# rrwick/Filtlong

Hardware: AMD Instinct MI355X
Metric: Mbases/s scored+sorted (higher is better)
Workload: dtype f64; 1 GPU; 10,000,000 synthetic reads per GPU x gamma(k=4) mean 10 kbp, Phred-only, --target_bases 50008889515 (50% of bases); C2; reads_total=10000000, bases_total=100017779031, window_size=250, parallelism=1 GPU, device=AMD Radeon Graphics (gfx950:sramecc+:xnack-), gpus_visible=1, cut=select

## Files before the change

filtlong_amd/csrc/score_phred_regs.hip:

```cpp
#include <algorithm>

#include "flx_internal.h"
#include "score_phred_common.h"

using namespace flx_phred;

#ifndef FLX_REGS_PART
#define FLX_REGS_PART 0
#endif

namespace {

template <bool PRIV>
struct Tab {
    static constexpr int ROW = PRIV ? 256 : 8;
    static constexpr int ENTRIES = PRIV ? 129 : LUT_PAD;
    static constexpr int BYTES = ROW * ENTRIES;
    static constexpr int QOFF = 0;
    static constexpr int DOFF = BYTES;
    static constexpr int ZIDX = PRIV ? 128 : 256;
    static constexpr int SLOT0 = 2 * BYTES;
};

template <bool PRIV, int SEL>
__device__ __forceinline__ uint32_t tab_addr(uint32_t x, uint32_t laneoff) {
    if (PRIV) {
        constexpr uint32_t sel = 0x0c0c0000u | ((4u + SEL) << 8);
        return __builtin_amdgcn_perm(x, laneoff, sel);
    }
    return lut_addr(x, SEL);
}
template <bool PRIV>
__device__ __forceinline__ uint32_t tab_addr_at(const uint32_t (&x)[8], int e, uint32_t laneoff) {
    switch (e & 3) {
        case 0: return tab_addr<PRIV, 0>(x[e >> 2], laneoff);
        case 1: return tab_addr<PRIV, 1>(x[e >> 2], laneoff);
        case 2: return tab_addr<PRIV, 2>(x[e >> 2], laneoff);
        default: return tab_addr<PRIV, 3>(x[e >> 2], laneoff);
    }
}

template <int QOFF, int DOFF>
__device__ __forceinline__ void fold4(uint32_t aj0, uint32_t aj1, uint32_t aj2, uint32_t aj3, uint32_t ai0, uint32_t ai1,
                                      uint32_t ai2, uint32_t ai3, double &s, double &w, double &mn) {
    double q0, i0, j0, q1, i1, j1, q2, i2, j2, q3, i3, j3;
    asm volatile(
        "ds_read_b64 %3, %15 offset:%23\n\tds_read_b64 %4, %19 offset:%24\n\tds_read_b64 %5, %15 offset:%24\n\t"
        "ds_read_b64 %6, %16 offset:%23\n\tds_read_b64 %7, %20 offset:%24\n\tds_read_b64 %8, %16 offset:%24\n\t"
        "ds_read_b64 %9, %17 offset:%23\n\tds_read_b64 %10, %21 offset:%24\n\tds_read_b64 %11, %17 offset:%24\n\t"
        "ds_read_b64 %12, %18 offset:%23\n\tds_read_b64 %13, %22 offset:%24\n\tds_read_b64 %14, %18 offset:%24\n\t"
        "s_waitcnt lgkmcnt(11)\n\tv_add_f64 %0, %0, %3\n\t"
        "s_waitcnt lgkmcnt(10)\n\tv_add_f64 %1, %1, -%4\n\t"
        "s_waitcnt lgkmcnt(9)\n\tv_add_f64 %1, %1, %5\n\tv_min_f64 %2, %2, %1\n\t"
        "s_waitcnt lgkmcnt(8)\n\tv_add_f64 %0, %0, %6\n\t"
        "s_waitcnt lgkmcnt(7)\n\tv_add_f64 %1, %1, -%7\n\t"
        "s_waitcnt lgkmcnt(6)\n\tv_add_f64 %1, %1, %8\n\tv_min_f64 %2, %2, %1\n\t"
        "s_waitcnt lgkmcnt(5)\n\tv_add_f64 %0, %0, %9\n\t"
        "s_waitcnt lgkmcnt(4)\n\tv_add_f64 %1, %1, -%10\n\t"
        "s_waitcnt lgkmcnt(3)\n\tv_add_f64 %1, %1, %11\n\tv_min_f64 %2, %2, %1\n\t"
        "s_waitcnt lgkmcnt(2)\n\tv_add_f64 %0, %0, %12\n\t"
        "s_waitcnt lgkmcnt(1)\n\tv_add_f64 %1, %1, -%13\n\t"
        "s_waitcnt lgkmcnt(0)\n\tv_add_f64 %1, %1, %14\n\tv_min_f64 %2, %2, %1"
        : "+v"(s), "+v"(w), "+v"(mn), "=&v"(q0), "=&v"(i0), "=&v"(j0), "=&v"(q1), "=&v"(i1), "=&v"(j1), "=&v"(q2), "=&v"(i2),
          "=&v"(j2), "=&v"(q3), "=&v"(i3), "=&v"(j3)
        : "v"(aj0), "v"(aj1), "v"(aj2), "v"(aj3), "v"(ai0), "v"(ai1), "v"(ai2), "v"(ai3), "i"(QOFF), "i"(DOFF));
}
template <int QOFF>
__device__ __forceinline__ void head4(uint32_t aj0, uint32_t aj1, uint32_t aj2, uint32_t aj3, double &s) {
    double q0, q1, q2, q3;
    asm volatile(
        "ds_read_b64 %1, %5 offset:%9\n\tds_read_b64 %2, %6 offset:%9\n\tds_read_b64 %3, %7 offset:%9\n\t"
        "ds_read_b64 %4, %8 offset:%9\n\t"
        "s_waitcnt lgkmcnt(3)\n\tv_add_f64 %0, %0, %1\n\ts_waitcnt lgkmcnt(2)\n\tv_add_f64 %0, %0, %2\n\t"
        "s_waitcnt lgkmcnt(1)\n\tv_add_f64 %0, %0, %3\n\ts_waitcnt lgkmcnt(0)\n\tv_add_f64 %0, %0, %4"
        : "+v"(s), "=&v"(q0), "=&v"(q1), "=&v"(q2), "=&v"(q3)
        : "v"(aj0), "v"(aj1), "v"(aj2), "v"(aj3), "i"(QOFF));
}
template <int QOFF>
__device__ __forceinline__ void head1(uint32_t aj, double &s) {
    double q;
    asm volatile("ds_read_b64 %1, %2 offset:%3\n\ts_waitcnt lgkmcnt(0)\n\tv_add_f64 %0, %0, %1" : "+v"(s), "=&v"(q) : "v"(aj), "i"(QOFF));
}
template <int QOFF, int DOFF>
__device__ __forceinline__ void fold1(uint32_t aj, uint32_t ai, double &s, double &w, double &mn) {
    double q, i, j;
    asm volatile(
        "ds_read_b64 %3, %6 offset:%8\n\tds_read_b64 %4, %7 offset:%9\n\tds_read_b64 %5, %6 offset:%9\n\t"
        "s_waitcnt lgkmcnt(2)\n\tv_add_f64 %0, %0, %3\n\ts_waitcnt lgkmcnt(1)\n\tv_add_f64 %1, %1, -%4\n\t"
        "s_waitcnt lgkmcnt(0)\n\tv_add_f64 %1, %1, %5\n\tv_min_f64 %2, %2, %1"
        : "+v"(s), "+v"(w), "+v"(mn), "=&v"(q), "=&v"(i), "=&v"(j)
        : "v"(aj), "v"(ai), "i"(QOFF), "i"(DOFF));
}

__device__ __forceinline__ void dma16(const void *gsrc, uint32_t lds_dst) {
    unsigned keep;
    asm volatile("s_mov_b32 %0, m0\n\ts_mov_b32 m0, %2\n\ts_nop 0\n\tglobal_load_lds_dwordx4 %1, off\n\ts_mov_b32 m0, %0"
                 : "=&s"(keep)
                 : "v"(gsrc), "s"(lds_dst)
                 : "memory");
}

__device__ __forceinline__ void funnel(const uint32_t (&p0)[4], const uint32_t (&p1)[4], int fD, uint32_t fsh, uint32_t (&tw)[4]) {
    const uint32_t x[8] = {p0[0], p0[1], p0[2], p0[3], p1[0], p1[1], p1[2], p1[3]};
#define FLX_FUN(D) _Pragma("unroll") for (int d = 0; d < 4; ++d) tw[d] = __builtin_amdgcn_alignbyte(x[(D) + d + 1], x[(D) + d], fsh);
    switch (fD) {
        case 0: FLX_FUN(0) break;
        case 1: FLX_FUN(1) break;
        case 2: FLX_FUN(2) break;
        case 3: FLX_FUN(3) break;
        default: tw[0] = x[4]; tw[1] = x[5]; tw[2] = x[6]; tw[3] = x[7]; break;
    }
#undef FLX_FUN
}

template <int A, bool PRIV, int WAVES, int BS = -1>
__global__ void __launch_bounds__(WAVES * 64) flx_score_phred_regs(const PhredArgs a) {
    using T = Tab<PRIV>;
    if (a.use_private && (*a.use_private != 0u) != PRIV) return;
    constexpr int R = ((A + 5 + 3) / 4) * 4;
    constexpr int RR = R / 4;
    constexpr int H = (A + 1 + 3) / 4;
    constexpr int SLOT_BYTES = 8192;
    static_assert(H <= RR, "prologue must fit one ring revolution");
    extern __shared__ __attribute__((aligned(16))) unsigned char smem[];

    if (PRIV) {
        for (int i = threadIdx.x; i < 129 * 32; i += WAVES * 64) {
            const int e = i >> 5;
            const double q = e < 128 ? a.lut_q[e] : 0.0, d = e < 128 ? a.lut_d[e] : 0.0;
            *reinterpret_cast<double *>(smem + T::QOFF + i * 8) = q;
            *reinterpret_cast<double *>(smem + T::DOFF + i * 8) = d;
        }
    } else {
        for (int i = threadIdx.x; i < 257; i += WAVES * 64) {
            *reinterpret_cast<double *>(smem + T::QOFF + i * 8) = a.lut_q[i];
            *reinterpret_cast<double *>(smem + T::DOFF + i * 8) = a.lut_d[i];
        }
    }
    __syncthreads();

    const int lane = threadIdx.x & 63;
    const int wave = threadIdx.x >> 6;
    unsigned char *slot = smem + T::SLOT0 + wave * SLOT_BYTES;
    const uint32_t slot_lds = (uint32_t)__builtin_amdgcn_readfirstlane((int)(T::SLOT0 + wave * SLOT_BYTES));
    const unsigned char *my_row = slot + lane * 64;
    const int rot = lane >> 2;
    const uint32_t laneoff = (uint32_t)(lane & 31) * 8u;
    const uint32_t zaddr = PRIV ? (uint32_t)(T::ZIDX * T::ROW) + laneoff : (uint32_t)(T::ZIDX * T::ROW);
    const int ws = a.ws;
    const int B = BS >= 0 ? BS : ws & 15;
    const int fD = (16 - B) >> 2;
    const uint32_t fsh = (uint32_t)(16 - B) & 3u;
    const double ws_d = a.ws_d;

  for (;;) {
    unsigned int group = 0;
    if (lane == 0) group = atomicAdd(a.ticket, 1u);
    group = (unsigned int)__builtin_amdgcn_readfirstlane((int)group);
    if (group >= a.n_groups) break;
    const uint64_t gslot = (uint64_t)group * 64 + lane;
    const bool slot_used = gslot < a.n_reads;
    uint32_t rid = 0;
    int L = 0;
    uint64_t base = 0;
    if (slot_used) {
        rid = a.order ? a.order[gslot] : (uint32_t)gslot;
        L = a.lengths[rid];
        base = a.offsets[rid];
    }
    const bool live = slot_used && L < a.long_thr;
    if (!live) L = 0;
    const int Lmax = wave_max(L);
    const int Lmin = wave_min(L);
    if (Lmax == 0) {
        if (live) finish_read(a, rid, L, 0.0, 0.0);
        continue;
    }
    const int n_rounds = (Lmax + 63) >> 6;

    const int dq = ((lane & 3) - (lane >> 4)) & 3;
    const uint8_t *gsrc[4];
    int lim[4];
#pragma unroll
    for (int m = 0; m < 4; ++m) {
        const int r = m * 16 + (lane >> 2);
        const uint32_t lo = __shfl((uint32_t)base, r, 64);
        const uint32_t hi = __shfl((uint32_t)(base >> 32), r, 64);
        gsrc[m] = a.plane + ((((uint64_t)hi << 32) | lo) + (uint64_t)(dq * 16));
        lim[m] = ((__shfl(L, r, 64) + 15) & ~15) - dq * 16;
    }
    auto issue_dma = [&](int c) {
        asm volatile("s_waitcnt lgkmcnt(0)" ::: "memory");
#pragma unroll
        for (int m = 0; m < 4; ++m) {
            const int o = c * 128;
            if (o < lim[m]) dma16(gsrc[m] + o, slot_lds + m * 1024);
            if (o + 64 < lim[m]) dma16(gsrc[m] + o + 64, slot_lds + 4096 + m * 1024);
        }
    };

    uint32_t ring[R][4];
#pragma unroll
    for (int i = 0; i < R; ++i) ring[i][0] = ring[i][1] = ring[i][2] = ring[i][3] = 0;
    double s = 0.0, w = 0.0, mn = 0.0;
    uint32_t bad = 0;

    auto load_round = [&](int t0, int r) {
        const int half = r & 1;
        if (half == 0) asm volatile("s_waitcnt vmcnt(0)" ::: "memory");
        const unsigned char *row = my_row + half * 4096;
#pragma unroll
        for (int k = 0; k < 4; ++k) {
            const uint4 v = *reinterpret_cast<const uint4 *>(row + (((k + rot) & 3) << 4));
            ring[t0 + k][0] = v.x; ring[t0 + k][1] = v.y; ring[t0 + k][2] = v.z; ring[t0 + k][3] = v.w;
            if (PRIV) bad |= v.x | v.y | v.z | v.w;
        }
        if (half == 1 && r + 1 < n_rounds) issue_dma((r + 1) >> 1);
    };
    auto mask4 = [&](bool masked, int rem, int k0, uint32_t (&o)[4]) {
        if (__builtin_expect(masked, 0)) {
#pragma unroll
            for (int i = 0; i < 4; ++i) o[i] = (k0 + i) < rem ? o[i] : zaddr;
        }
    };
    auto addr4 = [&](uint32_t x, bool masked, int rem, int k0, uint32_t (&o)[4]) {
        o[0] = tab_addr<PRIV, 0>(x, laneoff);
        o[1] = tab_addr<PRIV, 1>(x, laneoff);
        o[2] = tab_addr<PRIV, 2>(x, laneoff);
        o[3] = tab_addr<PRIV, 3>(x, laneoff);
        mask4(masked, rem, k0, o);
    };
    auto trail4_static = [&](const uint32_t (&p0)[4], const uint32_t (&p1)[4], int d, bool masked, int rem, uint32_t (&o)[4]) {
        const uint32_t x[8] = {p0[0], p0[1], p0[2], p0[3], p1[0], p1[1], p1[2], p1[3]};
#pragma unroll
        for (int i = 0; i < 4; ++i) o[i] = tab_addr_at<PRIV>(x, 16 - BS + 4 * d + i, laneoff);
        mask4(masked, rem, 4 * d, o);
    };
    auto head_piece = [&](const uint32_t (&lw)[4], int Tp) {
        const bool masked = 16 * (Tp + 1) > Lmin;
        const int rem = L - 16 * Tp;
#pragma unroll
        for (int d = 0; d < 4; ++d) {
            uint32_t aj[4];
            addr4(lw[d], masked, rem, 4 * d, aj);
            head4<T::QOFF>(aj[0], aj[1], aj[2], aj[3], s);
        }
    };
    auto steady_piece = [&](const uint32_t (&lw)[4], const uint32_t (&p0)[4], const uint32_t (&p1)[4], int Tp) {
        const bool masked = 16 * (Tp + 1) > Lmin;
        const int rem = L - 16 * Tp;
        uint32_t tw[4];
        if constexpr (BS < 0) funnel(p0, p1, fD, fsh, tw);
#pragma unroll
        for (int d = 0; d < 4; ++d) {
            uint32_t aj[4], ai[4];
            addr4(lw[d], masked, rem, 4 * d, aj);
            if constexpr (BS < 0) addr4(tw[d], masked, rem, 4 * d, ai);
            else trail4_static(p0, p1, d, masked, rem, ai);
            fold4<T::QOFF, T::DOFF>(aj[0], aj[1], aj[2], aj[3], ai[0], ai[1], ai[2], ai[3], s, w, mn);
        }
    };
    auto boundary_piece = [&](const uint32_t (&lw)[4], const uint32_t (&p0)[4], const uint32_t (&p1)[4], int Tp) {
        const int rem = L - 16 * Tp;
        uint32_t tw[4];
        if constexpr (BS < 0) funnel(p0, p1, fD, fsh, tw);
#pragma unroll
        for (int d = 0; d < 4; ++d) {
            uint32_t aj[4], ai[4];
            addr4(lw[d], true, rem, 4 * d, aj);
            if constexpr (BS < 0) addr4(tw[d], true, rem, 4 * d, ai);
            else trail4_static(p0, p1, d, true, rem, ai);
#pragma unroll
            for (int i = 0; i < 4; ++i) {
                const int k = 4 * d + i;
                if (k < B) head1<T::QOFF>(aj[i], s);
                else fold1<T::QOFF, T::DOFF>(aj[i], ai[i], s, w, mn);
                if (k == B - 1) {
                    w = s / ws_d;
                    mn = w;
                }
            }
        }
    };

    issue_dma(0);

#pragma unroll
    for (int h = 0; h < H; ++h) {
        if (h >= n_rounds) goto done;
        load_round(4 * h, h);
#pragma unroll
        for (int k = 0; k < 4; ++k) {
            constexpr int dummy = 0;
            (void)dummy;
            const int Tp = 4 * h + k;
            if (16 * Tp >= Lmax) continue;
            if (Tp < A) {
                head_piece(ring[Tp], Tp);
                if (Tp == A - 1 && B == 0) {
                    w = s / ws_d;
                    mn = w;
                }
            } else if (Tp == A) {
                boundary_piece(ring[Tp], ring[(Tp + R - A - 1) % R], ring[(Tp + R - A) % R], Tp);
            } else {
                steady_piece(ring[Tp], ring[(Tp + R - A - 1) % R], ring[(Tp + R - A) % R], Tp);
            }
        }
    }
    for (int rb = H;; rb += RR) {
#pragma unroll
        for (int u = 0; u < RR; ++u) {
            const int r = rb + u;
            if (r >= n_rounds) goto done;
            const int sr = (H + u) % RR;
            load_round(4 * sr, r);
#pragma unroll
            for (int k = 0; k < 4; ++k) {
                const int t = 4 * sr + k;
                const int Tp = 4 * r + k;
                if (16 * Tp >= Lmax) break;
                steady_piece(ring[t], ring[(t + R - A - 1) % R], ring[(t + R - A) % R], Tp);
            }
        }
    }
done:
    if (live) {
        finish_read(a, rid, L, s, mn);
        if (PRIV && (bad & 0x80808080u)) a.redo_list[atomicAdd(a.redo_count, 1u)] = rid;
    }
  }
}

#if FLX_REGS_PART == 0
__global__ void __launch_bounds__(1024) flx_score_phred_stream(const PhredArgs a) {
    using T = Tab<false>;
    extern __shared__ __attribute__((aligned(16))) unsigned char smem[];
    for (int i = threadIdx.x; i < 257; i += 1024) {
        *reinterpret_cast<double *>(smem + T::QOFF + i * 8) = a.lut_q[i];
        *reinterpret_cast<double *>(smem + T::DOFF + i * 8) = a.lut_d[i];
    }
    __syncthreads();
    const int lane = threadIdx.x & 63;
    const uint32_t zaddr = (uint32_t)(T::ZIDX * T::ROW);
    const int ws = a.ws;
    const int A = ws >> 4, B = ws & 15;
    const int fD = (16 - B) >> 2;
    const uint32_t fsh = (uint32_t)(16 - B) & 3u;
    const double ws_d = a.ws_d;
    for (;;) {
        unsigned int group = 0;
        if (lane == 0) group = atomicAdd(a.ticket, 1u);
        group = (unsigned int)__builtin_amdgcn_readfirstlane((int)group);
        if (group >= a.n_groups) break;
        const uint64_t gslot = (uint64_t)group * 64 + lane;
        const bool slot_used = gslot < a.n_reads;
        uint32_t rid = 0;
        int L = 0;
        uint64_t base = 0;
        if (slot_used) {
            rid = a.order ? a.order[gslot] : (uint32_t)gslot;
            L = a.lengths[rid];
            base = a.offsets[rid];
        }
        const bool live = slot_used && L < a.long_thr;
        if (!live) L = 0;
        const int Lmax = wave_max(L);
        if (Lmax == 0) {
            if (live) finish_read(a, rid, L, 0.0, 0.0);
            continue;
        }
        const uint8_t *src = (L > 0) ? a.plane + base : a.plane;
        const int maxoff = max(((L + 15) & ~15) - 16, 0);
        auto ld16 = [&](int off) { return *reinterpret_cast<const uint4 *>(src + min(max(off, 0), maxoff)); };
        const int n_pieces = (Lmax + 15) >> 4;
        double s = 0.0, w = 0.0, mn = 0.0;
        uint4 lead = ld16(0), lead_next = ld16(16);
        uint4 tr_prev = make_uint4(0, 0, 0, 0), tr_cur = tr_prev, tr_next = ld16(-16 * A);
        for (int t = 0; t < n_pieces; ++t) {
            const uint4 lw4 = lead;
            lead = lead_next;
            lead_next = ld16(16 * (t + 2));
            tr_prev = tr_cur;
            tr_cur = tr_next;
            tr_next = ld16(16 * (t + 1 - A));
            const uint32_t lw[4] = {lw4.x, lw4.y, lw4.z, lw4.w};
            const int rem = L - 16 * t;
            if (t < A) {
#pragma unroll
                for (int d = 0; d < 4; ++d) {
                    uint32_t aj[4];
                    aj[0] = tab_addr<false, 0>(lw[d], 0); aj[1] = tab_addr<false, 1>(lw[d], 0);
                    aj[2] = tab_addr<false, 2>(lw[d], 0); aj[3] = tab_addr<false, 3>(lw[d], 0);
#pragma unroll
                    for (int i = 0; i < 4; ++i) aj[i] = (4 * d + i) < rem ? aj[i] : zaddr;
                    head4<T::QOFF>(aj[0], aj[1], aj[2], aj[3], s);
                }
                if (t == A - 1 && B == 0) {
                    w = s / ws_d;
                    mn = w;
                }
                continue;
            }
            const uint32_t p0[4] = {tr_prev.x, tr_prev.y, tr_prev.z, tr_prev.w};
            const uint32_t p1[4] = {tr_cur.x, tr_cur.y, tr_cur.z, tr_cur.w};
            uint32_t tw[4];
            funnel(p0, p1, fD, fsh, tw);
#pragma unroll
            for (int d = 0; d < 4; ++d) {
                uint32_t aj[4], ai[4];
                aj[0] = tab_addr<false, 0>(lw[d], 0); aj[1] = tab_addr<false, 1>(lw[d], 0);
                aj[2] = tab_addr<false, 2>(lw[d], 0); aj[3] = tab_addr<false, 3>(lw[d], 0);
                ai[0] = tab_addr<false, 0>(tw[d], 0); ai[1] = tab_addr<false, 1>(tw[d], 0);
                ai[2] = tab_addr<false, 2>(tw[d], 0); ai[3] = tab_addr<false, 3>(tw[d], 0);
#pragma unroll
                for (int i = 0; i < 4; ++i) {
                    const bool act = (4 * d + i) < rem;
                    aj[i] = act ? aj[i] : zaddr;
                    ai[i] = act ? ai[i] : zaddr;
                }
                if (t > A) {
                    fold4<T::QOFF, T::DOFF>(aj[0], aj[1], aj[2], aj[3], ai[0], ai[1], ai[2], ai[3], s, w, mn);
                } else {
#pragma unroll
                    for (int i = 0; i < 4; ++i) {
                        const int k = 4 * d + i;
                        if (k < B) head1<T::QOFF>(aj[i], s);
                        else fold1<T::QOFF, T::DOFF>(aj[i], ai[i], s, w, mn);
                        if (k == B - 1) {
                            w = s / ws_d;
                            mn = w;
                        }
                    }
                }
            }
        }
        if (live) finish_read(a, rid, L, s, mn);
    }
}

constexpr int DUAL_WAVES = 9;
template <int AMOD>
__global__ void __launch_bounds__(DUAL_WAVES * 64) flx_score_phred_dual(const PhredArgs a) {
    using T = Tab<false>;
    constexpr int LEAD_BYTES = 8192, TRAIL_BYTES = 8192, WAVE_BYTES = LEAD_BYTES + TRAIL_BYTES;
    extern __shared__ __attribute__((aligned(16))) unsigned char smem[];
    for (int i = threadIdx.x; i < 257; i += DUAL_WAVES * 64) {
        *reinterpret_cast<double *>(smem + T::QOFF + i * 8) = a.lut_q[i];
        *reinterpret_cast<double *>(smem + T::DOFF + i * 8) = a.lut_d[i];
    }
    __syncthreads();
    const int lane = threadIdx.x & 63;
    const int wave = threadIdx.x >> 6;
    unsigned char *lead_slot = smem + T::SLOT0 + wave * WAVE_BYTES;
    unsigned char *trail_ring = lead_slot + LEAD_BYTES;
    const uint32_t lead_lds = (uint32_t)__builtin_amdgcn_readfirstlane((int)(T::SLOT0 + wave * WAVE_BYTES));
    const uint32_t trail_lds = lead_lds + LEAD_BYTES;
    const int rot = lane >> 2;
    const uint32_t zaddr = (uint32_t)(T::ZIDX * T::ROW);
    const int ws = a.ws;
    const int A = ws >> 4, B = ws & 15;
    const int A4 = A >> 2;
    const int fD = (16 - B) >> 2;
    const uint32_t fsh = (uint32_t)(16 - B) & 3u;
    const double ws_d = a.ws_d;

    for (;;) {
        unsigned int group = 0;
        if (lane == 0) group = atomicAdd(a.ticket, 1u);
        group = (unsigned int)__builtin_amdgcn_readfirstlane((int)group);
        if (group >= a.n_groups) break;
        const uint64_t gslot = (uint64_t)group * 64 + lane;
        const bool slot_used = gslot < a.n_reads;
        uint32_t rid = 0;
        int L = 0;
        uint64_t base = 0;
        if (slot_used) {
            rid = a.order ? a.order[gslot] : (uint32_t)gslot;
            L = a.lengths[rid];
            base = a.offsets[rid];
        }
        const bool live = slot_used && L < a.long_thr;
        if (!live) L = 0;
        const int Lmax = wave_max(L);
        const int Lmin = wave_min(L);
        if (Lmax == 0) {
            if (live) finish_read(a, rid, L, 0.0, 0.0);
            continue;
        }
        const int n_rounds = (Lmax + 63) >> 6;
        const int dq = ((lane & 3) - (lane >> 4)) & 3;
        const uint8_t *gsrc[4];
        int lim[4];
#pragma unroll
        for (int m = 0; m < 4; ++m) {
            const int r = m * 16 + (lane >> 2);
            const uint32_t lo = __shfl((uint32_t)base, r, 64);
            const uint32_t hi = __shfl((uint32_t)(base >> 32), r, 64);
            const int Lr = __shfl(L, r, 64);
            gsrc[m] = Lr > 0 ? a.plane + ((((uint64_t)hi << 32) | lo) + (uint64_t)(dq * 16)) : a.plane;
            lim[m] = Lr > 0 ? ((Lr + 15) & ~15) - dq * 16 : 0;
        }
        auto lds_idle = [&]() { asm volatile("s_waitcnt lgkmcnt(0)" ::: "memory"); };
        auto issue_lead = [&](int c) {
            lds_idle();
            const int o = c * 128;
#pragma unroll
            for (int m = 0; m < 4; ++m) {
                dma16(gsrc[m] + (o < lim[m] ? o : 0), lead_lds + m * 1024);
                dma16(gsrc[m] + (o + 64 < lim[m] ? o + 64 : 0), lead_lds + 4096 + m * 1024);
            }
        };
        auto issue_trail = [&](int h) {
            lds_idle();
            const int o = h * 64;
            const uint32_t dst = trail_lds + (uint32_t)(h & 1) * 4096u;
#pragma unroll
            for (int m = 0; m < 4; ++m) dma16(gsrc[m] + ((o >= 0 && o < lim[m]) ? o : 0), dst + m * 1024);
        };

        double s = 0.0, w = 0.0, mn = 0.0;
        uint32_t prev[4][4];
#pragma unroll
        for (int k = 0; k < 4; ++k) prev[k][0] = prev[k][1] = prev[k][2] = prev[k][3] = 0;
        issue_lead(0);
        if (A4 == 0) issue_trail(0);
        for (int r = 0; r < n_rounds; ++r) {
            const int h = r - A4;
            issue_trail(h + 1);
            asm volatile("s_waitcnt vmcnt(4)" ::: "memory");
            uint32_t lw[4][4], cur[4][4];
            const unsigned char *lrow = lead_slot + (r & 1) * 4096 + lane * 64;
            const unsigned char *trow = trail_ring + (h & 1) * 4096 + lane * 64;
#pragma unroll
            for (int k = 0; k < 4; ++k) {
                const uint4 v = *reinterpret_cast<const uint4 *>(lrow + (((k + rot) & 3) << 4));
                lw[k][0] = v.x; lw[k][1] = v.y; lw[k][2] = v.z; lw[k][3] = v.w;
            }
#pragma unroll
            for (int k = 0; k < 4; ++k) {
                uint4 v = make_uint4(0, 0, 0, 0);
                if (h >= 0) v = *reinterpret_cast<const uint4 *>(trow + (((k + rot) & 3) << 4));
                cur[k][0] = v.x; cur[k][1] = v.y; cur[k][2] = v.z; cur[k][3] = v.w;
            }
            if ((r & 1) && r + 1 < n_rounds) issue_lead((r + 1) >> 1);
#pragma unroll
            for (int k = 0; k < 4; ++k) {
                const int Tp = 4 * r + k;
                if (16 * Tp >= Lmax) break;
                const bool masked = 16 * (Tp + 1) > Lmin;
                const int rem = L - 16 * Tp;
                if (Tp < A) {
#pragma unroll
                    for (int d = 0; d < 4; ++d) {
                        uint32_t aj[4];
                        aj[0] = tab_addr<false, 0>(lw[k][d], 0); aj[1] = tab_addr<false, 1>(lw[k][d], 0);
                        aj[2] = tab_addr<false, 2>(lw[k][d], 0); aj[3] = tab_addr<false, 3>(lw[k][d], 0);
                        if (masked) {
#pragma unroll
                            for (int i = 0; i < 4; ++i) aj[i] = (4 * d + i) < rem ? aj[i] : zaddr;
                        }
                        head4<T::QOFF>(aj[0], aj[1], aj[2], aj[3], s);
                    }
                    if (Tp == A - 1 && B == 0) {
                        w = s / ws_d;
                        mn = w;
                    }
                    continue;
                }
                uint32_t tw[4];
                {
                    constexpr int dummy = 0;
                    (void)dummy;
                    const uint32_t(&p0)[4] = (k <= AMOD) ? prev[3 - AMOD + k] : cur[k - AMOD - 1];
                    const uint32_t(&p1)[4] = (k + 1 <= AMOD) ? prev[3 - AMOD + k + 1] : cur[k - AMOD];
                    funnel(p0, p1, fD, fsh, tw);
                }
#pragma unroll
                for (int d = 0; d < 4; ++d) {
                    uint32_t aj[4], ai[4];
                    aj[0] = tab_addr<false, 0>(lw[k][d], 0); aj[1] = tab_addr<false, 1>(lw[k][d], 0);
                    aj[2] = tab_addr<false, 2>(lw[k][d], 0); aj[3] = tab_addr<false, 3>(lw[k][d], 0);
                    ai[0] = tab_addr<false, 0>(tw[d], 0); ai[1] = tab_addr<false, 1>(tw[d], 0);
                    ai[2] = tab_addr<false, 2>(tw[d], 0); ai[3] = tab_addr<false, 3>(tw[d], 0);
                    if (masked || Tp == A) {
#pragma unroll
                        for (int i = 0; i < 4; ++i) {
                            const bool act = (4 * d + i) < rem;
                            aj[i] = act ? aj[i] : zaddr;
                            ai[i] = act ? ai[i] : zaddr;
                        }
                    }
                    if (Tp > A) {
                        fold4<T::QOFF, T::DOFF>(aj[0], aj[1], aj[2], aj[3], ai[0], ai[1], ai[2], ai[3], s, w, mn);
                    } else {
#pragma unroll
                        for (int i = 0; i < 4; ++i) {
                            const int kk = 4 * d + i;
                            if (kk < B) head1<T::QOFF>(aj[i], s);
                            else fold1<T::QOFF, T::DOFF>(aj[i], ai[i], s, w, mn);
                            if (kk == B - 1) {
                                w = s / ws_d;
                                mn = w;
                            }
                        }
                    }
                }
            }
#pragma unroll
            for (int k = 0; k < 4; ++k) {
                prev[k][0] = cur[k][0]; prev[k][1] = cur[k][1]; prev[k][2] = cur[k][2]; prev[k][3] = cur[k][3];
            }
        }
        asm volatile("s_waitcnt vmcnt(0)" ::: "memory");
        if (live) finish_read(a, rid, L, s, mn);
    }
}

__global__ void __launch_bounds__(256) flx_score_phred_redo(const PhredArgs a) {
    __shared__ double lq[LUT_PAD];
    __shared__ double ld[LUT_PAD];
    for (int i = threadIdx.x; i < 257; i += 256) {
        lq[i] = a.lut_q[i];
        ld[i] = a.lut_d[i];
    }
    __syncthreads();
    const unsigned int n = *a.redo_count;
    for (unsigned int i = blockIdx.x * 256 + threadIdx.x; i < n; i += gridDim.x * 256) {
        const uint32_t rid = a.redo_list[i];
        const int L = a.lengths[rid];
        const uint8_t *q = a.plane + a.offsets[rid];
        const int ws = a.ws;
        double s = 0.0, w = 0.0, mn = 0.0;
        const int head = L < ws ? L : ws;
        for (int j = 0; j < head; ++j) s += lq[q[j]];
        if (L > ws) {
            w = s / a.ws_d;
            mn = w;
            for (int j = ws; j < L; ++j) {
                const uint32_t cj = q[j], ci = q[j - ws];
                s += lq[cj];
                w -= ld[ci];
                w += ld[cj];
                if (w < mn) mn = w;
            }
        }
        finish_read(a, rid, L, s, mn);
    }
}

#endif

template <int A, bool PRIV, int WAVES, int BS = -1>
int launch_one(flx_ctx *ctx, PhredArgs &a) {
    using T = Tab<PRIV>;
    auto kern = flx_score_phred_regs<A, PRIV, WAVES, BS>;
    const size_t lds = std::max<size_t>((size_t)T::SLOT0 + (size_t)WAVES * 8192, 84 * 1024);
    FLX_HIP(ctx, hipFuncSetAttribute((const void *)kern, hipFuncAttributeMaxDynamicSharedMemorySize, (int)lds));
    const uint64_t per_block = (uint64_t)WAVES;
    const unsigned grid = (unsigned)std::min<uint64_t>(((uint64_t)a.n_groups + per_block - 1) / per_block,
                                                       (uint64_t)ctx->prop.multiProcessorCount);
    if (!a.use_private) {
        ctx->last_phred_kernel = PRIV ? "flx_score_phred_regs_private" : "flx_score_phred_regs";
        flx_time_begin(ctx, ctx->last_phred_kernel);
    }
    hipLaunchKernelGGL(kern, dim3(grid), dim3(WAVES * 64), lds, ctx->stream, a);
    if (!a.use_private) flx_time_end(ctx);
    FLX_HIP(ctx, hipGetLastError());
    return FLX_OK;
}

template <int A, bool PRIV>
struct WavesFor {
    static constexpr int plain = A <= 7 ? 16 : A <= 15 ? 12 : 8;
    static constexpr int value = PRIV && plain > 11 ? 11 : plain;
};

template <int A>
int launch_a(flx_ctx *ctx, PhredArgs &a, bool priv, int bs) {
    if constexpr (A == 15) {
        if (bs == 10) return priv ? launch_one<A, true, WavesFor<A, true>::value, 10>(ctx, a) : launch_one<A, false, WavesFor<A, false>::value, 10>(ctx, a);
    }
    if constexpr (A >= 32) {
        return launch_one<A, false, WavesFor<A, false>::value>(ctx, a);
    } else {
        return priv ? launch_one<A, true, WavesFor<A, true>::value>(ctx, a) : launch_one<A, false, WavesFor<A, false>::value>(ctx, a);
    }
}

template <int A, int A_END>
int launch_range(flx_ctx *ctx, PhredArgs &a, bool priv, int bs, bool *launched) {
    if constexpr (A < A_END) {
        if (a.ws / 16 != A) return launch_range<A + 1, A_END>(ctx, a, priv, bs, launched);
        *launched = true;
        return launch_a<A>(ctx, a, priv, bs);
    }
    return FLX_OK;
}

}

#define FLX_REGS_PARTS(X) X(0) X(1) X(2) X(3) X(4) X(5) X(6) X(7)
constexpr int kPartFirstA[] = {0, 8, 13, 18, 23, 28, 32, 36, 39};

#define FLX_REGS_PART_DECL(P) int flx_launch_score_phred_regs_part##P(flx_ctx *ctx, PhredArgs &a, bool priv, int bs, bool *launched);
FLX_REGS_PARTS(FLX_REGS_PART_DECL)
#define FLX_REGS_CAT2(a, b) a##b
#define FLX_REGS_CAT(a, b) FLX_REGS_CAT2(a, b)
int FLX_REGS_CAT(flx_launch_score_phred_regs_part, FLX_REGS_PART)(flx_ctx *ctx, PhredArgs &a, bool priv, int bs, bool *launched) {
    return launch_range<kPartFirstA[FLX_REGS_PART], kPartFirstA[FLX_REGS_PART + 1]>(ctx, a, priv, bs, launched);
}

#if FLX_REGS_PART == 0
namespace {
__global__ void __launch_bounds__(256) flx_phred_sample(const PhredArgs a, unsigned int *hist, unsigned int *done, unsigned int *use_private) {
    const uint64_t t = (uint64_t)blockIdx.x * 256 + threadIdx.x;
    uint64_t z = (t + 1) * 0x9E3779B97F4A7C15ULL;
    z = (z ^ (z >> 30)) * 0xBF58476D1CE4E5B9ULL;
    z = (z ^ (z >> 27)) * 0x94D049BB133111EBULL;
    z ^= z >> 31;
    const uint64_t r = z % a.n_reads;
    const int L = a.lengths[r];
    if (L > 0) {
        const uint32_t pos = (uint32_t)((z >> 32) % (uint64_t)L);
        atomicAdd(&hist[a.plane[a.offsets[r] + pos]], 1u);
    }
    __threadfence();
    __syncthreads();
    if (threadIdx.x != 0 || atomicAdd(done, 1u) != gridDim.x - 1) return;
    __threadfence();
    double tot = 0.0, conflicts = 0.0;
    bool high = false;
    for (int i = 0; i < 256; ++i) {
        const unsigned int h = __hip_atomic_load(&hist[i], __ATOMIC_RELAXED, __HIP_MEMORY_SCOPE_AGENT);
        tot += h;
        high = high || (i >= 128 && h != 0);
    }
    if (tot > 0) {
        for (int b = 0; b < 32; ++b) {
            double pb = 0.0, sq = 0.0;
            for (int e = b; e < 256; e += 32) {
                const double pe = __hip_atomic_load(&hist[e], __ATOMIC_RELAXED, __HIP_MEMORY_SCOPE_AGENT) / tot;
                pb += pe;
                sq += pe * pe;
            }
            conflicts += pb * pb - sq;
        }
    }
    *use_private = (!high && 496.0 * conflicts > 3.0) ? 1u : 0u;
}

}

int flx_launch_score_phred_stream(flx_ctx *ctx, PhredArgs a) {
    void *scr;
    FLX_CHECK(flx_scratch(ctx, 64, &scr));
    FLX_HIP(ctx, hipMemsetAsync(scr, 0, 8, ctx->stream));
    a.ticket = (unsigned int *)scr;
    a.n_groups = (unsigned int)((a.n_reads + 63) / 64);
    const size_t lds = 84 * 1024;
    FLX_HIP(ctx, hipFuncSetAttribute((const void *)flx_score_phred_stream, hipFuncAttributeMaxDynamicSharedMemorySize, (int)lds));
    const unsigned grid = (unsigned)std::min<uint64_t>(((uint64_t)a.n_groups + 15) / 16, (uint64_t)ctx->prop.multiProcessorCount);
    ctx->last_phred_kernel = "flx_score_phred_stream";
    flx_time_begin(ctx, ctx->last_phred_kernel);
    hipLaunchKernelGGL(flx_score_phred_stream, dim3(grid), dim3(1024), lds, ctx->stream, a);
    flx_time_end(ctx);
    FLX_HIP(ctx, hipGetLastError());
    return FLX_OK;
}

int flx_launch_score_phred_dual(flx_ctx *ctx, PhredArgs a) {
    void *scr;
    FLX_CHECK(flx_scratch(ctx, 64, &scr));
    FLX_HIP(ctx, hipMemsetAsync(scr, 0, 8, ctx->stream));
    a.ticket = (unsigned int *)scr;
    a.n_groups = (unsigned int)((a.n_reads + 63) / 64);
    const size_t lds = (size_t)Tab<false>::SLOT0 + (size_t)DUAL_WAVES * 16384;
    const unsigned grid = (unsigned)std::min<uint64_t>(((uint64_t)a.n_groups + DUAL_WAVES - 1) / DUAL_WAVES, (uint64_t)ctx->prop.multiProcessorCount);
    ctx->last_phred_kernel = "flx_score_phred_dual";
    flx_time_begin(ctx, ctx->last_phred_kernel);
#define FLX_DUAL_LAUNCH(M)                                                                                                              \
    case M:                                                                                                                             \
        FLX_HIP(ctx, hipFuncSetAttribute((const void *)flx_score_phred_dual<M>, hipFuncAttributeMaxDynamicSharedMemorySize, (int)lds)); \
        hipLaunchKernelGGL(flx_score_phred_dual<M>, dim3(grid), dim3(DUAL_WAVES * 64), lds, ctx->stream, a);                            \
        break;
    switch ((a.ws >> 4) & 3) {
        FLX_DUAL_LAUNCH(0) FLX_DUAL_LAUNCH(1) FLX_DUAL_LAUNCH(2) FLX_DUAL_LAUNCH(3)
    }
#undef FLX_DUAL_LAUNCH
    flx_time_end(ctx);
    FLX_HIP(ctx, hipGetLastError());
    return FLX_OK;
}

int flx_launch_score_phred_regs(flx_ctx *ctx, PhredArgs a, bool *launched, PhredPending *pd) {
    *launched = false;
    const int A = a.ws / 16;
    constexpr int n_parts = (int)(sizeof kPartFirstA / sizeof kPartFirstA[0]) - 1;
    if (A >= kPartFirstA[n_parts]) return FLX_OK;
    const char *env = getenv("FLX_PHRED_TABLES");
    bool priv = env && strcmp(env, "private") == 0;
    bool forced = env && (strcmp(env, "private") == 0 || strcmp(env, "plain") == 0);
    if (A >= 32) {
        forced = true;
        priv = false;
    }
    const char *fenv = getenv("FLX_PHRED_FUNNEL");
    if (fenv && *fenv && strcmp(fenv, "runtime") != 0)
        return flx_fail(ctx, FLX_ERR_INVALID, "FLX_PHRED_FUNNEL=%s: expected runtime (or unset)", fenv);
    const int bs = (a.ws == 250 && !(fenv && *fenv)) ? 10 : -1;
    void *scr;
    FLX_CHECK(flx_scratch(ctx, 2048 + a.n_reads * 4, &scr));
    a.ticket = (unsigned int *)scr;
    a.redo_count = (unsigned int *)scr + 1;
    a.redo_list = (uint32_t *)((char *)scr + 2048);
    unsigned int *d_flag = (unsigned int *)scr + 3;
    FLX_HIP(ctx, hipMemsetAsync(scr, 0, 2048, ctx->stream));
    if (!forced) {
        hipLaunchKernelGGL(flx_phred_sample, dim3(64), dim3(256), 0, ctx->stream, a, (unsigned int *)((char *)scr + 64),
                           (unsigned int *)scr + 2, d_flag);
        a.use_private = d_flag;
    }
    a.n_groups = (unsigned int)((a.n_reads + 63) / 64);
    typedef int (*part_fn)(flx_ctx *, PhredArgs &, bool, int, bool *);
#define FLX_REGS_PART_NAME(P) flx_launch_score_phred_regs_part##P,
    static const part_fn parts[n_parts] = {FLX_REGS_PARTS(FLX_REGS_PART_NAME)};
#undef FLX_REGS_PART_NAME
    int P = 0;
    while (A >= kPartFirstA[P + 1]) ++P;
    auto part = [&](bool pv) { return parts[P](ctx, a, pv, bs, launched); };
    long timed_index = -1;
    if (forced) {
        FLX_CHECK(part(priv));
    } else {
        ctx->last_phred_kernel = "flx_score_phred_regs";
        flx_time_scope t(ctx, ctx->last_phred_kernel);
        if (ctx->timing) timed_index = (long)ctx->timed.size() - 1;
        FLX_CHECK(part(false));
        FLX_CHECK(part(true));
    }
    if (!*launched) return FLX_OK;
    if (priv || !forced) {
        flx_time_begin(ctx, "flx_score_phred_redo");
        hipLaunchKernelGGL(flx_score_phred_redo, dim3(256), dim3(256), 0, ctx->stream, a);
        flx_time_end(ctx);
        FLX_HIP(ctx, hipGetLastError());
    }
    if (!forced) {
        pd->chosen_on_device = true;
        pd->timed_index = timed_index;
        FLX_HIP(ctx, hipMemcpyAsync(pd->h_flag, d_flag, 4, hipMemcpyDeviceToHost, ctx->stream));
    }
    return FLX_OK;
}
#endif
```

Before: 3.473 million Mbases/s.

## Remap per-lane DMA pieces to eight 16-byte loads via LDS pointer table

Replaces the four-read-by-four-piece DMA mapping, which needed 64-bit shuffles of each read's base address and limit, with an eight-read-by-eight-piece mapping. Each lane's read base pointer is now kept in a small per-wave LDS pointer table. A fast path skips the per-piece bounds check when every read in the wave is long enough for the current chunk. The LDS read side uses an XOR-swizzled layout verified by constexpr asserts. This cuts shuffle and register pressure in the DMA issue, at the cost of extra LDS traffic for pointer loads and a little more LDS per wave.

```diff
diff --git a/filtlong_amd/csrc/phred_dma_map.h b/filtlong_amd/csrc/phred_dma_map.h
--- /dev/null
+++ b/filtlong_amd/csrc/phred_dma_map.h
@@ -0,0 +1,27 @@
+#pragma once
+
+namespace flx_phred_dma {
+
+constexpr int SLOT_BYTES = 8192;
+constexpr int N_DMA = 8;
+
+constexpr int read_of(int m, int l) { return 8 * m + (l >> 3); }
+constexpr int row_pos(int R, int p) { return (p + (R >> 1)) & 7; }
+constexpr int piece_of(int m, int l) { return ((l & 7) - (read_of(m, l) >> 1)) & 7; }
+constexpr int piece_even(int l) { return ((l & 7) - (l >> 4)) & 7; }
+constexpr int landing(int m, int l) { return 1024 * m + 16 * l; }
+constexpr int lane_read(int R, int p) { return 128 * R + 16 * row_pos(R, p); }
+
+
+constexpr bool shortcuts_hold() {
+    for (int m = 0; m < N_DMA; ++m)
+        for (int l = 0; l < 64; ++l)
+            if (piece_of(m, l) != (piece_even(l) ^ (4 * (m & 1)))) return false;
+    for (int R = 0; R < 64; ++R)
+        for (int p = 0; p < 4; ++p)
+            if (lane_read(R, p + 4) != (lane_read(R, p) ^ 64)) return false;
+    return true;
+}
+static_assert(shortcuts_hold(), "piece_even / the ^ 64 of the second half do not match the map");
+
+}
diff --git a/filtlong_amd/csrc/score_phred_regs.hip b/filtlong_amd/csrc/score_phred_regs.hip
--- a/filtlong_amd/csrc/score_phred_regs.hip
+++ b/filtlong_amd/csrc/score_phred_regs.hip
@@ -1,6 +1,7 @@
 #include <algorithm>
 
 #include "flx_internal.h"
+#include "phred_dma_map.h"
 #include "score_phred_common.h"
 
 using namespace flx_phred;
@@ -21,6 +22,8 @@
     static constexpr int ZIDX = PRIV ? 128 : 256;
     static constexpr int SLOT0 = 2 * BYTES;
 };
+constexpr int REGS_PTR_BYTES = 64 * 8;
+constexpr int REGS_WAVE_BYTES = flx_phred_dma::SLOT_BYTES + REGS_PTR_BYTES;
 
 template <bool PRIV, int SEL>
 __device__ __forceinline__ uint32_t tab_addr(uint32_t x, uint32_t laneoff) {
@@ -120,7 +123,7 @@
     constexpr int R = ((A + 5 + 3) / 4) * 4;
     constexpr int RR = R / 4;
     constexpr int H = (A + 1 + 3) / 4;
-    constexpr int SLOT_BYTES = 8192;
+    constexpr int SLOT_BYTES = flx_phred_dma::SLOT_BYTES;
     static_assert(H <= RR, "prologue must fit one ring revolution");
     extern __shared__ __attribute__((aligned(16))) unsigned char smem[];
 
@@ -143,8 +146,7 @@
     const int wave = threadIdx.x >> 6;
     unsigned char *slot = smem + T::SLOT0 + wave * SLOT_BYTES;
     const uint32_t slot_lds = (uint32_t)__builtin_amdgcn_readfirstlane((int)(T::SLOT0 + wave * SLOT_BYTES));
-    const unsigned char *my_row = slot + lane * 64;
-    const int rot = lane >> 2;
+    const uint8_t **ptab = reinterpret_cast<const uint8_t **>(smem + T::SLOT0 + WAVES * SLOT_BYTES + wave * REGS_PTR_BYTES);
     const uint32_t laneoff = (uint32_t)(lane & 31) * 8u;
     const uint32_t zaddr = PRIV ? (uint32_t)(T::ZIDX * T::ROW) + laneoff : (uint32_t)(T::ZIDX * T::ROW);
     const int ws = a.ws;
@@ -178,24 +180,31 @@
     }
     const int n_rounds = (Lmax + 63) >> 6;
 
-    const int dq = ((lane & 3) - (lane >> 4)) & 3;
-    const uint8_t *gsrc[4];
-    int lim[4];
-#pragma unroll
-    for (int m = 0; m < 4; ++m) {
-        const int r = m * 16 + (lane >> 2);
-        const uint32_t lo = __shfl((uint32_t)base, r, 64);
-        const uint32_t hi = __shfl((uint32_t)(base >> 32), r, 64);
-        gsrc[m] = a.plane + ((((uint64_t)hi << 32) | lo) + (uint64_t)(dq * 16));
-        lim[m] = ((__shfl(L, r, 64) + 15) & ~15) - dq * 16;
-    }
+    const int Lpad = (L + 15) & ~15;
+    const int Lpad_min = (Lmin + 15) & ~15;
+    ptab[lane] = a.plane + base;
     auto issue_dma = [&](int c) {
         asm volatile("s_waitcnt lgkmcnt(0)" ::: "memory");
-#pragma unroll
-        for (int m = 0; m < 4; ++m) {
-            const int o = c * 128;
-            if (o < lim[m]) dma16(gsrc[m] + o, slot_lds + m * 1024);
-            if (o + 64 < lim[m]) dma16(gsrc[m] + o + 64, slot_lds + 4096 + m * 1024);
+        int ln = lane;
+        asm volatile("" : "+v"(ln));
+        const uint32_t oe = (uint32_t)c * 128u + 16u * (uint32_t)flx_phred_dma::piece_even(ln), oo = oe ^ 64u;
+        const uint8_t **prow = ptab + flx_phred_dma::read_of(0, ln);
+        static_assert(flx_phred_dma::read_of(1, 0) == 8 && flx_phred_dma::read_of(7, 63) == 63, "prow[8 m], 4 * r0 + 32 m below");
+        if (128 * (c + 1) <= Lpad_min) {
+            const uint8_t *next = prow[0];
+#pragma unroll
+            for (int m = 0; m < flx_phred_dma::N_DMA; ++m) {
+                const uint8_t *src = next;
+                if (m + 1 < flx_phred_dma::N_DMA) next = prow[8 * (m + 1)];
+                dma16(src + ((m & 1) ? oo : oe), slot_lds + (uint32_t)flx_phred_dma::landing(m, 0));
+            }
+        } else {
+            const int r0x4 = 4 * flx_phred_dma::read_of(0, ln);
+#pragma unroll
+            for (int m = 0; m < flx_phred_dma::N_DMA; ++m) {
+                const uint32_t o = (m & 1) ? oo : oe;
+                if ((int)o < __builtin_amdgcn_ds_bpermute(r0x4 + 32 * m, Lpad)) dma16(prow[8 * m] + o, slot_lds + (uint32_t)flx_phred_dma::landing(m, 0));
+            }
         }
     };
 
@@ -208,10 +217,9 @@
     auto load_round = [&](int t0, int r) {
         const int half = r & 1;
         if (half == 0) asm volatile("s_waitcnt vmcnt(0)" ::: "memory");
-        const unsigned char *row = my_row + half * 4096;
 #pragma unroll
         for (int k = 0; k < 4; ++k) {
-            const uint4 v = *reinterpret_cast<const uint4 *>(row + (((k + rot) & 3) << 4));
+            const uint4 v = *reinterpret_cast<const uint4 *>(slot + (flx_phred_dma::lane_read(lane, k) ^ (half << 6)));
             ring[t0 + k][0] = v.x; ring[t0 + k][1] = v.y; ring[t0 + k][2] = v.z; ring[t0 + k][3] = v.w;
             if (PRIV) bad |= v.x | v.y | v.z | v.w;
         }
@@ -655,7 +663,8 @@
 int launch_one(flx_ctx *ctx, PhredArgs &a) {
     using T = Tab<PRIV>;
     auto kern = flx_score_phred_regs<A, PRIV, WAVES, BS>;
-    const size_t lds = std::max<size_t>((size_t)T::SLOT0 + (size_t)WAVES * 8192, 84 * 1024);
+    const size_t lds = std::max<size_t>((size_t)T::SLOT0 + (size_t)WAVES * REGS_WAVE_BYTES, 84 * 1024);
+    static_assert((size_t)T::SLOT0 + (size_t)WAVES * REGS_WAVE_BYTES <= 160 * 1024, "tables, slots and address tables must fit the LDS");
     FLX_HIP(ctx, hipFuncSetAttribute((const void *)kern, hipFuncAttributeMaxDynamicSharedMemorySize, (int)lds));
     const uint64_t per_block = (uint64_t)WAVES;
     const unsigned grid = (unsigned)std::min<uint64_t>(((uint64_t)a.n_groups + per_block - 1) / per_block,
```

After: 3.452 million Mbases/s. About the same (-0.6%).
